# bab2min/Kiwi

Measured on AMD Instinct MI355X. Metric: sentences/sec on batched analyze(), device kernels with inputs resident in HBM (dictionary scan + lattice + Viterbi/Knlm, top-1); host-to-host rate: see e2e, higher is better.
Workload: dtype int32+f32; 1 GPU; c2-64k: 65536 synthetic sentences ({'exact_jamo': 40}), synthetic 'full' model (kiwi_amd/synth.py), Knlm, top-1; sentences_per_gpu=65536, chunks_per_gpu=65536, jamo_per_gpu=2621440, parallelism=shard1, device_bytes=9547378333, rerun_chunks=0

## Files before the change

### kiwi_amd/csrc/device_types.hpp

```cpp
#pragma once
#include <cstdint>
#include "flat_model.hpp"

namespace kamd
{
	struct DevPattern { uint32_t end, length; uint32_t tag; };
	constexpr uint32_t kSpanTag = 0x80000000u, kSpanFallback = 0x40000000u, kSpanFormMask = 0x00FFFFFFu;

	struct alignas(16) DevNode
	{
		uint32_t form;
		uint16_t startPos, endPos;
		uint16_t prev, sibling;
		uint16_t uformOff, uformLen;
		uint8_t spaceErrors;
		uint8_t nflags;
		uint16_t nPrev;
		uint32_t packOff;
		uint16_t candCnt;
		uint8_t fflags;
		uint8_t flen;
		uint16_t ownFeat;
		uint16_t pad;
	};
// ... 125 lines not shown
		const uint32_t* packBase;
		CandStatic* packs;
		const uint64_t* tokenBase;
		DevToken* tokens;
		DevChunkResult* results;
		DevPathHeader* outPaths;
		DevToken* outTokens;
		uint32_t* outCounters;
		uint32_t* wideList;
		uint8_t* expanded;
		float* unkChr;
		float* unkChrForm;
		const uint32_t* blockBits;
		uint32_t outPathCap, outTokCap;
		PosRec* posRecs; PosDesc* posDesc; uint32_t* posPrev; uint32_t* posNodeRec; uint32_t* posMask;
		uint8_t* posBig;
		uint8_t* posScratch; uint32_t* posContCounter; uint32_t posContSlots;
		uint32_t* posHandOver;
		uint8_t* bigScratch;
		uint32_t bigScratchBytes;
		uint32_t* beacon;
	};

	struct SbgDev
	{
		const uint32_t* ptrs;
		const uint32_t* keys;
		const float* comps;
		const float* discnts;
		const uint8_t* valid;
		uint32_t vocabSize; float logWindowSize;
// ... 87 lines not shown
```

### kiwi_amd/csrc/engine.hip

```cpp
#include <hip/hip_runtime.h>
#include <unistd.h>
#include <cstdio>
#include <cstring>
#include <ctime>
#include <algorithm>
#include <atomic>
#include <cstdlib>
#include <chrono>
#include <condition_variable>
#include <functional>
#include <map>
#include <mutex>
#include <numeric>
#include <stdexcept>
#include <thread>
#include "engine.hpp"
#include "pretok.hpp"
#include "hostpool.hpp"
#include "post_fast.hpp"
#include "viterbi_kernel.hpp"
#include "exact_math.hpp"
#include "cong_global.hpp"
#include "chr_freq.hpp"
#include "typo_lattice_kernel.hpp"
// ... 160 lines not shown
		uint64_t units = 0, devBytes = 0;
		std::vector<uint32_t> charOff, patOff, spOff, matchBase, nodeBase, packBase;
		std::vector<uint64_t> stateBase, tokenBase;
		PinBuf hIn; DevBuf dIn;
		DevBuf dFullMask, dZAt, dNsToPos, dPosToNs, dCflag, dMask, dMoff, dNNs, dMatchForm, dNodes, dTmpNodes, dEndPosMap, dTmpIdx, dNNodes, dWideList, dExpanded;
		struct LatClass { uint32_t i, j, need, stream; };
		std::vector<std::vector<LatClass>> latClasses; std::vector<uint32_t> latSkip; uint32_t latClassesKey = 0xFFFFFFFFu;
		DevBuf dHist;
		uint32_t slotCap = 0; uint64_t ownStates = 0;
		DevBuf dStateAt, dSlotTable; uint64_t poolStates = 0, poolUsed = 0;
		TypoOption typo;
		TypoGraphDev typoDev;
		DevBuf dTypoGraph, dTypoLast, dTypoPool, dTypoChunks, dTypoTmp, dTypoMap, dTypoNs, dTypoPs, dTypoStates, dTypoSIdx, dTypoScratch, dNodeTypo, dTypoOrder, dBlockBits, dUnkChr, dUnkChrForm;
		TypoLatView tv{};
		DevBuf dPacks, dStates, dNodeStOff, dNodeStCnt, dReach, dTokens, dResults, dOrder;
		DevBuf dPosRecs, dPosDesc, dPosPrev, dPosNodeRec, dPosMask, dPosBig;
		DevBuf dOutPaths, dOutTokens, dOutCounters; uint32_t outPathCap = 0, outTokCap = 0;
		PinBuf hOut, hOut2;
		uint64_t outBytes = 0;
		BatchView bv{}; WorkView wv{};
		const DevChunkResult* hResults = nullptr; const DevPathHeader* hPaths = nullptr; const DevToken* hTokens = nullptr; size_t hTokCount = 0;
		bool ran = false;
		hipEvent_t evDone = nullptr; bool launched = false; uint32_t launchS = 1;
		~StagedBatch()
		{
			if (evDone) (void)hipEventDestroy(evDone);
			if (prepBlocks.size() >= 64)
			{
				try { HostPool::instance().run(prepBlocks.size(), 16, hostThreads, [&](size_t i0, size_t i1, int) { for (size_t i = i0; i < i1; ++i) { PrepBlock dead = std::move(prepBlocks[i]); } }); }
				catch (...) {}
			}
// ... 427 lines not shown
		b.poolStates = tinyArenas ? 0 : slotMode ? (I.poolForced ? ownStates * I.poolFrac64 / 64 : ownStates / 4)
			: std::max<uint64_t>(ownStates * I.poolFrac64 / 64, I.poolFrac64 ? std::min<uint64_t>(ownStates, 1u << 16) : 0);
		b.ownStates = ownStates;
		const uint64_t totStates = ownStates + b.poolStates, totTokens = b.tokenBase[nC];
		b.dNsToPos.ensure(perChar * 2); b.dPosToNs.ensure(perChar * 2); b.dCflag.ensure(perChar); b.dMask.ensure(perChar * 8); b.dMoff.ensure(perChar * 4);
		b.dNNs.ensure(nC * 4 + 16); b.dMatchForm.ensure(totMatch * 4 + 16);
		b.dNodes.ensure(totNodes * sizeof(DevNode) + 16); b.dTmpNodes.ensure(totNodes * sizeof(DevNode) + 16);
		b.dEndPosMap.ensure(perChar * 4); b.dFullMask.ensure(perChar * 8); b.dZAt.ensure(perChar); b.dTmpIdx.ensure(totNodes * 4 + 16); b.dNNodes.ensure(nC * 4 + 16); b.dWideList.ensure(nC * 4 + 16); b.dExpanded.ensure(nC + 16);
		b.dPacks.ensure((size_t)b.packBase[nC] * sizeof(CandStatic) + 16);
		b.dStates.ensure(totStates * sizeof(DevState) + 16); b.dNodeStOff.ensure(totNodes * 4 + 16); b.dNodeStCnt.ensure(totNodes * 4 + 16); b.dReach.ensure(totNodes + 16);
		b.dTokens.ensure(totTokens * sizeof(DevToken) + 16); b.dResults.ensure(nC * sizeof(DevChunkResult) + 16);
		const bool posPath = I.posPath && !I.histStates();
		if (posPath)
		{
			b.dPosRecs.ensure((size_t)b.packBase[nC] * sizeof(PosRec) + 16); b.dPosDesc.ensure(totNodes * sizeof(PosDesc) + 16);
			b.dPosPrev.ensure(totNodes * 4 + 16); b.dPosNodeRec.ensure(totNodes * 4 + 16); b.dPosMask.ensure(totNodes * (b.typo.typo ? 8 : 4) + 16) ; b.dPosBig.ensure(((nC + 7) / 8 * 8) * (size_t)64 * 20 + 16);
		}
		if (I.histStates()) b.dHist.ensure(totStates * 32 + 32);
		b.outTokCap = (uint32_t)std::min<uint64_t>(totTokens, 0xFFFFFFF0ull); b.outPathCap = (uint32_t)std::min<uint64_t>((uint64_t)nC * 16 * sc, 0xFFFFFFF0ull);
		b.dOutTokens.ensure((size_t)b.outTokCap * sizeof(DevToken) + 16); b.dOutPaths.ensure((size_t)b.outPathCap * sizeof(DevPathHeader) + 16); b.dOutCounters.ensure(128);
		b.dStateAt.ensure(nC * 8 + 16); if (slotMode) b.dSlotTable.ensure((size_t)I.histSlots() * 16 + 16);
		b.devBytes = 0;
		for (const DevBuf* d : { &b.dIn, &b.dOutTokens, &b.dOutPaths, &b.dNsToPos, &b.dPosToNs, &b.dCflag, &b.dMask, &b.dMoff, &b.dMatchForm, &b.dNodes, &b.dTmpNodes, &b.dEndPosMap, &b.dTmpIdx,
			&b.dPacks, &b.dStates, &b.dHist, &b.dStateAt, &b.dSlotTable, &b.dNodeStOff, &b.dNodeStCnt, &b.dReach, &b.dTokens, &b.dResults, &b.dPosRecs, &b.dPosDesc, &b.dPosPrev, &b.dPosNodeRec, &b.dPosMask, &b.dPosBig }) b.devBytes += d->cap;

		BatchView& bv = b.bv;
		bv.nChunks = (uint32_t)nC; bv.chars = (const uint16_t*)(D + oChars); bv.cls = D + oCls; bv.script = D + oScript;
		bv.charOff = (const uint32_t*)(D + oCharOff); bv.patOff = (const uint32_t*)(D + oPatOff); bv.patterns = (const DevPattern*)(D + oPats);
		bv.spOff = (const uint32_t*)(D + oSpOff); bv.spStates = D + oSp; bv.chunkFlags = D + oFlags; bv.textOffset = (const uint32_t*)(D + oTextOff);
		bv.filtChars = chrFreq ? (const uint16_t*)(D + oFilt) : nullptr; bv.filtOff = chrFreq ? (const uint32_t*)(D + oFiltOff) : nullptr; bv.filtLen = chrFreq ? (const uint32_t*)(D + oFiltLen) : nullptr;
		WorkView& w = b.wv;
		w.nsToPos = b.dNsToPos.as<uint16_t>(); w.posToNs = b.dPosToNs.as<uint16_t>(); w.cflag = b.dCflag.as<uint8_t>();
		w.matchMask = b.dMask.as<uint64_t>(); w.matchOff = b.dMoff.as<uint32_t>(); w.nNs = b.dNNs.as<uint32_t>();
		w.matchBase = (const uint32_t*)(D + oMatchBase); w.matchForm = b.dMatchForm.as<uint32_t>();
		w.nodeBase = (const uint32_t*)(D + oNodeBase); w.nodes = b.dNodes.as<DevNode>(); w.tmpNodes = b.dTmpNodes.as<DevNode>();
		w.endPosMap = b.dEndPosMap.as<uint32_t>(); w.fullMask = b.dFullMask.as<uint64_t>(); w.zAt = b.dZAt.as<uint8_t>(); w.tmpIdx = b.dTmpIdx.as<uint16_t>(); w.nNodes = b.dNNodes.as<uint32_t>(); w.wideList = b.dWideList.as<uint32_t>(); w.expanded = b.dExpanded.as<uint8_t>();
		w.packBase = (const uint32_t*)(D + oPackBase); w.packs = b.dPacks.as<CandStatic>();
		w.stateBase = (const uint64_t*)(D + oStateBase); w.states = b.dStates.as<DevState>();
		w.stateAt = b.dStateAt.as<uint64_t>(); w.poolTop = b.poolStates ? reinterpret_cast<unsigned long long*>(b.dOutCounters.as<uint32_t>() + 16) : nullptr;
		w.poolBase = b.ownStates; w.poolCap = b.poolStates; w.slotCap = b.slotCap; w.slotTable = b.slotCap ? b.dSlotTable.as<uint64_t>() : nullptr;
		w.nodeStateOff = b.dNodeStOff.as<uint32_t>(); w.nodeStateCnt = b.dNodeStCnt.as<uint32_t>(); w.reach = b.dReach.as<uint8_t>();
		w.tokenBase = (const uint64_t*)(D + oTokenBase); w.tokens = b.dTokens.as<DevToken>(); w.results = b.dResults.as<DevChunkResult>();
		w.outTokens = b.dOutTokens.as<DevToken>(); w.outPaths = b.dOutPaths.as<DevPathHeader>(); w.outCounters = b.dOutCounters.as<uint32_t>();
		w.outTokCap = b.outTokCap; w.outPathCap = b.outPathCap;
		w.posRecs = posPath ? b.dPosRecs.as<PosRec>() : nullptr; w.posDesc = posPath ? b.dPosDesc.as<PosDesc>() : nullptr;
		w.posPrev = posPath ? b.dPosPrev.as<uint32_t>() : nullptr; w.posNodeRec = posPath ? b.dPosNodeRec.as<uint32_t>() : nullptr; w.posMask = posPath ? b.dPosMask.as<uint32_t>() : nullptr; w.posBig = posPath ? b.dPosBig.as<uint8_t>() : nullptr;
		w.posHandOver = nullptr; w.posScratch = nullptr; w.posContCounter = nullptr; w.posContSlots = 0;
		w.blockBits = nullptr;
		w.unkChr = nullptr;
		w.unkChrForm = nullptr;
		if ((b.match >> 8) & 3) { b.dUnkChr.ensure(totNodes * 4 + 16); w.unkChr = b.dUnkChr.as<float>(); }
		if (((b.match >> 8) & 3) > 1) { b.dUnkChrForm.ensure(totNodes * 4 + 16); w.unkChrForm = b.dUnkChrForm.as<float>(); }
		if (b.typo.blocked && !b.typo.blocked->empty() && b.typo.blocked->size() != (I.model.morphs.size() + 31) / 32) throw std::invalid_argument{ "kiwi_amd: blocklist bit set does not belong to this model" };
		const size_t nTempMorphs = b.pretok ? b.pretok->temps.morphs.size() : 0;
		if (!I.model.morphDialect.empty() || (nTempMorphs && b.typo.blocked && !b.typo.blocked->empty()))
		{
			std::vector<uint32_t>& bits = b.blockBitsHost;
			bits.assign((I.model.morphs.size() + 31) / 32, 0u);
			if (b.typo.blocked && !b.typo.blocked->empty()) bits = *b.typo.blocked;
			bool any = b.typo.blocked && !b.typo.blocked->empty();
			for (size_t i = 0; i < I.model.morphDialect.size(); ++i) { const uint32_t d = I.model.morphDialect[i]; if (d && !(d & b.typo.allowedDialect)) { bits[i >> 5] |= 1u << (i & 31); any = true; } }
// ... 1762 lines not shown
```

### kiwi_amd/csrc/viterbi_pos.inc

```
#if !defined(KAMD_SBG) && !defined(KAMD_CONGG)
	template<int G> struct PosCaps
	{
#ifdef KAMD_TEST_SMALL_CAPS
		static constexpr uint32_t PST_CAP = 8;
#else
		static constexpr uint32_t PST_CAP = G == 16 ? 64 : 32;
#endif
		static constexpr uint32_t PHR = G == 16 ? 32 : 16;
	};
	constexpr uint32_t PBIG_CAP = 64;
	struct PosBigItem { uint32_t keyLo, keyHi; float score, fcs; uint32_t ctx; };
	struct PosGroupCtx { uint64_t st, recs, uniq, nodeTypo; uint32_t stCap, stTop, posStart, ringTop, firstRec, retry, ofNodes, bigBase; };
	static_assert(sizeof(PosGroupCtx) == 64, "PosGroupCtx");
	template<int G> struct PosLayT
	{
		static constexpr uint32_t PST_CAP = PosCaps<G>::PST_CAP, PHR = PosCaps<G>::PHR;
		static constexpr uint32_t RBEG = 0, REND = 4 * RING, RCUM = 8 * RING;
		static constexpr uint32_t NCNT = 12 * RING;
		static constexpr uint32_t ACUR = NCNT + 4 * G, ALAST = ACUR + 32, ATMP = ALAST + 32;
		static constexpr uint32_t GCTX = ATMP + 32;
		static constexpr uint32_t RINFO = GCTX + 64;
		static constexpr uint32_t PBEST = RINFO;
		static constexpr uint32_t OVFL = RINFO + 4 * G;
		static constexpr uint32_t RECS = OVFL + 16;
		static constexpr uint32_t STSC = RECS + G * 48;
		static constexpr uint32_t STB = STSC + 4 * PST_CAP;
		static constexpr uint32_t HOTR = (STB + 2 * PST_CAP + 15) & ~15u;
// ... 2 lines not shown
		static constexpr uint32_t CTXR = TYPR + 4 * PHR, SIZE = (CTXR + 4 * PHR + 15) & ~15u;
#else
		static constexpr uint32_t CHR = TYPR + 4 * PHR, SIZE = (CHR + 8 * PHR + 15) & ~15u;
#endif
		static constexpr uint32_t ROWMAP = (64 / G) * SIZE, TOTAL = ROWMAP + 128;
	};
#if defined(KAMD_TYPO)
	constexpr uint32_t kPosLds16 = kPosKernelLdsBytes + 4 * kTypoRingExtra, kPosLds8 = kPosKernelLdsBytes8 + 8 * kTypoRingExtra;
#else
	constexpr uint32_t kPosLds16 = kPosKernelLdsBytes, kPosLds8 = kPosKernelLdsBytes8;
#endif
	static_assert(PosLayT<16>::TOTAL <= kPosLds16 && PosLayT<8>::TOTAL <= kPosLds8, "k_pos_path LDS");
	static_assert(Lay<16>::TOTAL <= kPosLds16 && Lay<16>::TOTAL <= kPosLds8, "k_pos_path LDS: the general search carrying on in the kernel");
	enum : uint32_t { PSB_PASS1 = 0x1000 };
#if defined(KAMD_POSSTATS) && defined(KAMD_HIPEMU)
	struct PosStats { std::atomic<unsigned long long> c[24]; ~PosStats() { fprintf(stderr, "[posstats] waveSteps %llu groupSteps %llu rounds %llu bigRounds %llu itemLanes %llu deadParents %llu scored %llu kept %llu multiChunkItems %llu roundsWithMulti %llu argmaxIters %llu reps %llu lmCalls %llu retries %llu rowsUsed %llu zItems %llu sockItems %llu testSteps %llu testChunks %llu\n",
		c[0].load(), c[1].load(), c[2].load(), c[3].load(), c[4].load(), c[5].load(), c[6].load(), c[7].load(), c[8].load(), c[9].load(), c[10].load(), c[11].load(), c[12].load(), c[13].load(), c[14].load(), c[15].load(), c[16].load(), c[17].load(), c[18].load()); } };
	static PosStats gPosStats;
	struct PosHist { std::atomic<unsigned long long> h[6][70]; ~PosHist() { static const char* nm[6] = { "nRec", "nodes", "newStates", "itemsPerRecord", "parentAge", "nodeDist" }; for (int a = 0; a < 6; ++a) { fprintf(stderr, "[poshist] %s:", nm[a]); for (int b = 0; b < 70; ++b) if (h[a][b].load()) fprintf(stderr, " %d:%llu", b, h[a][b].load()); fprintf(stderr, "\n"); } } };
	static PosHist gPosHist;
#define PHIST(a, v) gPosHist.h[a][(v) < 69u ? (v) : 69u]++;
#define PSTAT(k, n) gPosStats.c[k] += (n);
#else
#define PSTAT(k, n) (void)0;
#define PHIST(a, v) (void)0;
#endif

	__device__ __forceinline__ uint32_t rowOr16(uint32_t v) { v |= rowRor<8>(v); v |= rowRor<4>(v); v |= rowRor<2>(v); v |= rowRor<1>(v); return v; }
	__device__ __forceinline__ uint32_t rowMaxU16(uint32_t v)
	{
		uint32_t o;
		o = rowRor<8>(v); v = o > v ? o : v; o = rowRor<4>(v); v = o > v ? o : v; o = rowRor<2>(v); v = o > v ? o : v; o = rowRor<1>(v); v = o > v ? o : v;
// ... 70 lines not shown
		return true;
	}

	template<int G, int WPS>
	__global__ void __launch_bounds__(64, WPS) k_pos_path(ModelView M, BatchView B, WorkView W, SearchParams P, const uint32_t* chunkOrder, uint32_t nWork TYPO_ONLY(, const float* nodeTypoAll) CONG_ONLY(, CongDev CGv))
	{
		static_assert(G == 16 || G == 8, "a lane group is one DPP row or half of one");
		using PosLay = PosLayT<G>;
		constexpr uint32_t NG = 64 / G, GM = (1u << G) - 1u, PST_CAP = PosLay::PST_CAP, PHR = PosLay::PHR;
#ifdef KAMD_TYPO
		constexpr uint32_t kP = 2;
#else
		constexpr uint32_t kP = 16 / G;
#endif
		const uint32_t lane = threadIdx.x, gl = lane & (uint32_t)(G - 1), gshift = lane & (uint32_t)(64 - G), grp = lane / (uint32_t)G, lds = grp * PosLay::SIZE;
		const uint32_t il = lane & 15u, ishift = lane & 48u, irow = lane >> 4; (void)ishift;
		LDS_AS uint32_t* rBeg = ldsPtr<uint32_t>(lds + PosLay::RBEG);
		LDS_AS uint32_t* rEnd = ldsPtr<uint32_t>(lds + PosLay::REND);
		LDS_AS uint32_t* rCum = ldsPtr<uint32_t>(lds + PosLay::RCUM);
		LDS_AS uint32_t* nCnt = ldsPtr<uint32_t>(lds + PosLay::NCNT);
		LDS_AS uint32_t* aCur = ldsPtr<uint32_t>(lds + PosLay::ACUR);
		LDS_AS uint32_t* aLast = ldsPtr<uint32_t>(lds + PosLay::ALAST);
		LDS_AS uint32_t* aTmp = ldsPtr<uint32_t>(lds + PosLay::ATMP);
		LDS_AS uint32_t* gctx = ldsPtr<uint32_t>(lds + PosLay::GCTX);
		LDS_AS uint32_t* rinfo = ldsPtr<uint32_t>(lds + PosLay::RINFO);
		LDS_AS uint32_t* ovfL = ldsPtr<uint32_t>(lds + PosLay::OVFL);
		LDS_AS uint16_t* rowMap = ldsPtr<uint16_t>(PosLay::ROWMAP);
		rowMap[lane] = 0;
		auto tbit = [](LDS_AS uint32_t* a, uint32_t x) -> uint32_t { return (a[(x >> 5) & 7u] >> (x & 31u)) & 1u; };
		auto sbit = [](LDS_AS uint32_t* a, uint32_t x) { a[(x >> 5) & 7u] |= 1u << (x & 31u); };
		LDS_AS float* typR = ldsPtr<float>(lds + PosLay::TYPR);
#ifdef KAMD_CONG
		LDS_AS uint32_t* ctxR = ldsPtr<uint32_t>(lds + PosLay::CTXR);
#else
		LDS_AS uint32_t* chR = ldsPtr<uint32_t>(lds + PosLay::CHR);
#endif
		const uint32_t hotR = lds + PosLay::HOTR;
		LDS_AS float* stSc = ldsPtr<float>(lds + PosLay::STSC);
		LDS_AS uint16_t* stB = ldsPtr<uint16_t>(lds + PosLay::STB);
#define GBALLOT(p) ((uint32_t)((__ballot(p) >> gshift) & GM))
#define GSHFL(v, l) __shfl((v), (int)(l), G)
#ifdef KAMD_HIPEMU
#define WBALLOT(p) hipemu_ballot64(p)
#define WSHFL(v, l) hipemu_shfl64((v), (int)(l))
#define WREADLANE(v, l) hipemu_shfl64((v), (int)(l))
#define ISHFL16(v, l) hipemu_shfl64((v), (int)(ishift + ((uint32_t)(l) & 15u)))
#define IROR(N, v) ((uint32_t)hipemu_row_ror64((int)(v), (N)))
#define IRORF(N, v) __uint_as_float((uint32_t)hipemu_row_ror64((int)__float_as_uint(v), (N)))
#else
#define WBALLOT(p) ((unsigned long long)__ballot(p))
#define WSHFL(v, l) __shfl((v), (int)(l), 64)
#define WREADLANE(v, l) ((uint32_t)__builtin_amdgcn_readlane((int)(v), (int)(l)))
#define ISHFL16(v, l) __shfl((v), (int)(l), 16)
#define IROR(N, v) rowRor<N>(v)
#define IRORF(N, v) rowRorF<N>(v)
#endif
#define IBALLOT16(p) ((uint32_t)((WBALLOT(p) >> ishift) & 0xFFFFu))
#ifdef KAMD_POS_DEBUG
#define PBEACON(code, a, b2, c2) { if (W.beacon && mine && gl == 0) { uint32_t* bq_ = W.beacon + 64ull * chunk; __builtin_nontemporal_store((uint32_t)(code), bq_); __builtin_nontemporal_store((uint32_t)(a), bq_ + 1); __builtin_nontemporal_store((uint32_t)(b2), bq_ + 2); __builtin_nontemporal_store((uint32_t)(c2), bq_ + 3); } }
		unsigned long long tlLast = clock64(); uint32_t tlAcc[14] = { 0, 0, 0, 0, 0, 0, 0, 0, 0, 0, 0, 0, 0, 0 };
#define PTL(k) { const unsigned long long t_ = clock64(); tlAcc[k] += (uint32_t)(t_ - tlLast); tlLast = t_; }
#else
#define PBEACON(code, a, b2, c2)
#define PTL(k)
#endif
		const unsigned long long lowerMask64 = (1ull << lane) - 1ull;

		const uint32_t ci = blockIdx.x * NG + grp;
		const bool mine = ci < nWork;
		const uint32_t chunk = mine ? chunkOrder[ci] : chunkOrder[0];
		DevChunkResult* res = &W.results[chunk];
		bool active = mine && res->status == CS_OK;
		if (mine && !active && gl == 0) res->nPaths = 0;
		const bool searching = active;
		PBEACON(1, ci, 0, 0)
		const uint32_t nBase = W.nodeBase[chunk];
		const uint32_t Gn = W.nNodes[chunk];
		DevState* st = W.states + W.stateBase[chunk];
		const uint32_t stCap = (uint32_t)(W.stateBase[chunk + 1] - W.stateBase[chunk]);
		uint32_t* nodeStOff = W.nodeStateOff + nBase; uint32_t* nodeStCnt = W.nodeStateCnt + nBase; uint16_t* nodeLive = W.tmpIdx + 2ull * nBase;
		const uint8_t* uniq = B.spStates + B.spOff[chunk];
// ... 181 lines not shown
#endif
				if (active)
				{
					rinfo[gl] = pBegRp[0] | ((rqp[0] & 0xFFu) << 27);
					if (gl < nRec) { ldsStore4(lds + PosLay::RECS + 48 * gl, rec0); ldsStore4(lds + PosLay::RECS + 48 * gl + 16, rec1); ldsStore4(lds + PosLay::RECS + 48 * gl + 32, rec2); }
					if (gl == 0)
					{
						LDS_AS uint64_t* g64 = (LDS_AS uint64_t*)gctx;
						g64[0] = (uint64_t)st; g64[1] = (uint64_t)(recs + firstRec); g64[2] = (uint64_t)uniq; g64[3] = (uint64_t)nodeTypo;
						gctx[8] = stCap; gctx[9] = stTop; gctx[10] = stTop; gctx[11] = ringTop; gctx[12] = 0; gctx[13] = retry0 | (retry1 << 16);
#ifdef KAMD_CONG
						gctx[14] = ofNodes;
#else
						gctx[14] = 0;
#endif
						gctx[15] = (blockIdx.x * NG + grp) * PBIG_CAP;
						*ovfL = 0;
					}
					posStart = stTop;
				}
				PTL(1)
			}
			__syncthreads();

			for (uint32_t pass = 0; pass < kP; ++pass)
			{
			if (pass)
			{
				if (!WBALLOT(active && nRec > (uint32_t)G)) break;
				if (active)
				{
// ... 8 lines not shown
			}
			const uint32_t Qw = active ? ((kP > 1 && pass) ? Qp[kP - 1] : Qp[0]) : 0u;

			{
				uint32_t S16 = Qw;
				{ uint32_t t; t = IROR(1, S16); S16 += il >= 1 ? t : 0u; t = IROR(2, S16); S16 += il >= 2 ? t : 0u; t = IROR(4, S16); S16 += il >= 4 ? t : 0u; t = IROR(8, S16); S16 += il >= 8 ? t : 0u; }
				const uint32_t T0 = WREADLANE(S16, 15), T1 = WREADLANE(S16, 31), T2 = WREADLANE(S16, 47);
				const uint32_t Winc = S16 + (irow >= 1 ? T0 : 0u) + (irow >= 2 ? T1 : 0u) + (irow >= 3 ? T2 : 0u);
				const unsigned long long nzAll = WBALLOT(Qw != 0);
				uint32_t recDoneW = 0, baseW = 0, guardW = 0;
				while (recDoneW < 64)
				{
					const unsigned long long nz = nzAll & ~((1ull << recDoneW) - 1ull);
					if (!nz) break;
					if (++guardW > 80u) { *ovfL = 1; break; }
					const uint32_t first = (uint32_t)__ffsll((unsigned long long)nz) - 1u;
					const uint32_t Qfirst = WREADLANE(Qw, first);
					const bool bigMode = Qfirst > 16u;
					int myRow = -1; uint32_t myStart = 0, nRows = 0, myItemsRow = 0;
					if (bigMode) { recDoneW = first + 1; baseW = WREADLANE(Winc, first); }
					else
					{
						for (uint32_t b = 0; b < 4; ++b)
						{
							const bool take = lane >= recDoneW && Winc - baseW <= 16u;
							const unsigned long long tm = WBALLOT(take);
							const uint32_t n = (uint32_t)__popcll(tm);
							if (!n) break;
							if (take) { myRow = (int)b; myStart = Winc - Qw - baseW; }
							const uint32_t it = WREADLANE(Winc, recDoneW + n - 1) - baseW;
							if (irow == b) myItemsRow = it;
							baseW += it; recDoneW += n; nRows = b + 1;
							if (recDoneW >= 64) break;
						}
					}
					PTL(2)
					if (lane == 0) { PSTAT(2, 1) PSTAT(3, bigMode ? 1 : 0) PSTAT(14, bigMode ? 4 : nRows) }
					const uint32_t q = bigMode ? lane : il;
					bool valid; uint32_t recLane, local, lastK = 0;
					if (!bigMode)
					{
						if (myRow >= 0 && Qw) rowMap[16 * (uint32_t)myRow + myStart] = (uint16_t)((lane | (myStart << 8) | ((Qw - 1u) << 12)) + 1u);
						__syncthreads();
						valid = irow < nRows && il < myItemsRow;
						uint32_t e = rowMap[lane];
						rowMap[lane] = 0;
						{ uint32_t o;
						  o = IROR(1, e); e = (e == 0 && il >= 1) ? o : e;
						  o = IROR(2, e); e = (e == 0 && il >= 2) ? o : e;
						  o = IROR(4, e); e = (e == 0 && il >= 4) ? o : e;
						  o = IROR(8, e); e = (e == 0 && il >= 8) ? o : e; }
						e = e ? e - 1u : 0u;
						recLane = valid ? (e & 0xFFu) : lane;
						local = valid ? il - ((e >> 8) & 15u) : 0u;
						lastK = valid ? ((e >> 8) & 15u) + (e >> 12) : il;
					}
					else { valid = lane < Qfirst; recLane = valid ? first : lane; local = lane; }
					const uint32_t startK = q - local;
					const uint32_t owner = recLane / (uint32_t)G, k = recLane & (uint32_t)(G - 1), ldsO = owner * PosLay::SIZE;
					const uint4 g0 = ldsLoad4(ldsO + PosLay::GCTX), g1 = ldsLoad4(ldsO + PosLay::GCTX + 16), g2 = ldsLoad4(ldsO + PosLay::GCTX + 32), g3 = ldsLoad4(ldsO + PosLay::GCTX + 48);
					DevState* stO = reinterpret_cast<DevState*>((uint64_t)g0.x | ((uint64_t)g0.y << 32));
					const uint8_t* uniqO = reinterpret_cast<const uint8_t*>((uint64_t)g1.x | ((uint64_t)g1.y << 32));
					const float* nodeTypoO = reinterpret_cast<const float*>((uint64_t)g1.z | ((uint64_t)g1.w << 32)); (void)nodeTypoO;
					const uint32_t stCapO = g2.x, stTopO = g2.y, posStartO = g2.z, ringTopO = g2.w;
					const uint32_t retry0O = g3.y & 0xFFFFu, retry1O = g3.y >> 16, bigBaseO = g3.w;
					CONG_ONLY(const uint32_t ofNodesO = g3.z;)
					const uint32_t ri = ldsPtr<uint32_t>(ldsO + PosLay::RINFO)[k];
					const uint32_t pBegK = ri & 0x7FFFFFFu, R = ri >> 27;
					const uint32_t hotRO = ldsO + PosLay::HOTR;
					LDS_AS float* typRO = ldsPtr<float>(ldsO + PosLay::TYPR);
#ifdef KAMD_CONG
					LDS_AS uint32_t* ctxRO = ldsPtr<uint32_t>(ldsO + PosLay::CTXR);
#else
					LDS_AS uint32_t* chRO = ldsPtr<uint32_t>(ldsO + PosLay::CHR);
#endif
					LDS_AS float* stScO = ldsPtr<float>(ldsO + PosLay::STSC);
					LDS_AS uint16_t* stBO = ldsPtr<uint16_t>(ldsO + PosLay::STB);
					uint4 ra = make_uint4(0, 0, 0, 0), rb = ra, rc = ra;
					if (valid) { ra = ldsLoad4(ldsO + PosLay::RECS + 48 * k); rb = ldsLoad4(ldsO + PosLay::RECS + 48 * k + 16); rc = ldsLoad4(ldsO + PosLay::RECS + 48 * k + 32); }
					Cand c;
// ... 5 lines not shown
					const uint8_t ownKind = (uint8_t)(rc.z >> 16), nflags = (uint8_t)(rc.z >> 24);
					const uint32_t nl = (rc.w >> 8) & 0xFFu;
					const bool spaceBefore = nflags & NF_SPACE_BEFORE;
					const bool isZ = (rc.w & PR_Z) != 0;
					uint32_t p = local, r = 0;
					if (R > 1) { p = local / R; r = local % R; }

					PTL(3)
					float cand = 0, firstChunk = 0, rTypo = 0; int32_t lmNode = 0; uint8_t rootKey = 0, sp = 0;
					CONG_ONLY(uint32_t ctx = 0;)
					CONG_ONLY(uint32_t pctx = 0;)
#ifndef KAMD_CONG
					uint32_t pch1 = 0, pch2 = 0, nch1 = 0, nch2 = 0;
#endif
					if (valid) PSTAT(4, 1)
					if (valid)
					{
						const uint32_t pidx = pBegK + p, slot = pidx & (PHR - 1);
						PHIST(4, ringTopO - pidx)
						Hot ps;
						if (ringTopO - pidx <= PHR)
						{
							const uint4 a = ldsLoad4(hotRO + 16 * slot);
							ps.lmNode = (int32_t)a.x; ps.accScore = __uint_as_float(a.y); ps.w2 = a.z; ps.w3 = a.w;
							rTypo = typRO[slot];
#ifdef KAMD_CONG
							pctx = ctxRO[slot];
#else
							pch1 = chRO[2 * slot]; pch2 = chRO[2 * slot + 1];
#endif
						}
						else
						{
							ps = loadHot(stO, pidx);
							rTypo = stO[pidx].accTypoCost;
#ifdef KAMD_CONG
							pctx = stO[pidx].pad0;
#else
							const uint2 pc = *reinterpret_cast<const uint2*>(&stO[pidx].pad0); pch1 = pc.x; pch2 = pc.y;
#endif
						}
						const bool single = c.single();
						const uint8_t ctag = c.tag(), csock = c.socket();
						uint32_t firstWid = c.firstWid; bool widReplaced = false;
#ifdef KAMD_POS_DEBUG
						if (ps.accScore == 12345.678f && c.additional == 9876.5f) tlAcc[0] += 1;
						PTL(12)
#endif
// ... 97 lines not shown
#endif
							sp = ps.spState();
							rootKey = ps.rootId();
							if (c.quoteOrBullet())
							{
								if (rootKey == COMMON_ROOT) sp = uniqO[r];
								else if (r != 0) { valid = false; break; }
							}
							const float rs = ruleScore(c, ps.prevFlags(), sp);
							cand = cand + rs; firstChunk = firstChunk + rs;
							if (c.ruleBits & RB_DIALECT) { cand = cand - P.dialectCost; firstChunk = firstChunk - P.dialectCost; }
							sp = nextSpState(c, sp);
						} while (0);
					}
					PTL(4)
					if (valid) PSTAT(7, 1)
					const uint64_t rKey = valid ? ((uint64_t)(uint32_t)lmNode | ((uint64_t)sp << 32) | ((uint64_t)rootKey << 40) | ((uint64_t)recLane << 48)) : KINVALID;
					const float rScore = cand, rFcs = firstChunk;

					auto emitState = [&](uint32_t pos, bool ring, int32_t wNode, uint8_t wSp, uint8_t wRoot, float wscore, float wfcs, float wtyp, uint32_t wx1, uint32_t wx2, uint32_t wl)
					{
						const uint32_t rslot = pos & (PHR - 1);
						uint32_t parent = pBegK + wl, wr = 0;
						if (R != 1) { parent = pBegK + wl / R; wr = wl % R; }
						const uint32_t rel = pos - posStartO;
						if (isZ)
						{
							const uint4* ps4 = reinterpret_cast<const uint4*>(stO + parent);
							const uint4 a = ps4[0], b2 = ps4[1], c2 = ps4[2];
							const uint16_t lfMorph = (uint16_t)c.chunkOff; const uint8_t nmPrevFlags = (uint8_t)(c.chunkOff >> 16); const bool newMorphSocket = (c.chunkOff >> 24) & 1u;
// ... 44 lines not shown
							ctxRO[rslot] = wx1;
#else
							chRO[2 * rslot] = wx1; chRO[2 * rslot + 1] = wx2;
#endif
						}
#ifdef KAMD_CONG
						(void)wx2;
#else
						*reinterpret_cast<uint2*>(&stO[pos].pad0) = make_uint2(wx1, wx2);
#endif
						stScO[rel] = wscore;
						stBO[rel] = (uint16_t)((newRoot == COMMON_ROOT ? 0u : newRoot + 1u) | (c.socket() ? (uint32_t)SB_MORPH_SOCKET : 0u) | (stSocket ? (uint32_t)SB_STATE_SOCKET : 0u)
							| (nl << 8) | ((rc.w & PR_PASS1) ? (uint32_t)PSB_PASS1 : 0u));
					};
					const uint32_t keyLo = (uint32_t)rKey, keyHi = (uint32_t)(rKey >> 32);
					bool rep; float best, wfcs, wtyp; uint32_t wl, wx1, wx2, wNodeU, wHi;
					if (!bigMode)
					{
						rep = false; best = rScore; uint32_t qw = q;
						const uint32_t recMask = ((2u << (lastK - startK)) - 1u) << startK;
						bool un = valid;
						while (WBALLOT(un))
						{
							if (lane == 0) PSTAT(10, 1)
							const uint32_t mine = IBALLOT16(un) & recMask;
							const uint32_t f = mine ? (uint32_t)__ffs((int)mine) - 1u : q;
							const uint32_t kLo = ISHFL16(keyLo, f), kHi = ISHFL16(keyHi, f);
							const bool match = un & (keyLo == kLo) & (keyHi == kHi);
							float bs = match ? rScore : -3.0e38f; uint32_t bi = q;
#define KAMD_POS_SEG(N) { const float os = IRORF(N, bs); const uint32_t oi = IROR(N, bi); const bool take = (q >= startK + N) & (os >= bs); bs = take ? os : bs; bi = take ? oi : bi; }
							KAMD_POS_SEG(1) KAMD_POS_SEG(2) KAMD_POS_SEG(4) KAMD_POS_SEG(8)
#undef KAMD_POS_SEG
							const float rb = ISHFL16(bs, lastK); const uint32_t rq = ISHFL16(bi, lastK);
							if (match && q == f) { rep = true; best = rb; qw = rq; }
							un = un && !match;
						}
						PTL(5)
						wfcs = ISHFL16(rFcs, qw);
						wtyp = ISHFL16(rTypo, qw);
#ifdef KAMD_CONG
						wx1 = ISHFL16(ctx, qw); wx2 = 0;
#else
						wx1 = nch1; wx2 = nch2;
#endif
						wl = qw - startK; wNodeU = (uint32_t)lmNode; wHi = keyHi;
					}
					else
					{
						PosBigItem* big = reinterpret_cast<PosBigItem*>(W.posBig) + bigBaseO;
						if (lane < Qfirst)
						{
							PosBigItem it; it.keyLo = keyLo; it.keyHi = keyHi; it.score = rScore; it.fcs = rFcs;
#ifdef KAMD_CONG
							it.ctx = ctx;
#else
							it.ctx = 0;
#endif
							big[lane] = it;
						}
						__syncthreads();
						rep = false; best = 0; uint32_t qw = lane;
						if (lane < Qfirst && (keyLo & keyHi) != 0xFFFFFFFFu)
						{
							rep = true; bool have = false;
							for (uint32_t j = 0; j < Qfirst; ++j)
							{
								if (big[j].keyLo != keyLo || big[j].keyHi != keyHi) continue;
								if (j < lane) { rep = false; break; }
								const float sj = big[j].score;
								if (!have || sj > best) { best = sj; qw = j; have = true; }
							}
						}
						wfcs = 0; wtyp = 0; wx1 = 0; wx2 = 0;
						if (rep)
						{
							wfcs = big[qw].fcs;
							wtyp = stO[pBegK + (R > 1 ? qw / R : qw)].accTypoCost;
#ifdef KAMD_CONG
							wx1 = big[qw].ctx;
#else
							if (!isZ) { const uint2 nc = *reinterpret_cast<const uint2*>(M.lmChain + 2 * (size_t)keyLo); wx1 = nc.x; wx2 = nc.y; }
#endif
						}
						wl = qw; wNodeU = keyLo; wHi = keyHi;
						__syncthreads();
					}
					uint32_t myRank = 0, myAdd = 0, ownerAdd = 0;
					for (uint32_t g2i = 0; g2i < NG; ++g2i)
					{
						const unsigned long long bg = WBALLOT(rep && owner == g2i);
						if (owner == g2i) { myRank = (uint32_t)__popcll(bg & lowerMask64); ownerAdd = (uint32_t)__popcll(bg); }
						if (grp == g2i) myAdd = (uint32_t)__popcll(bg);
					}
					if (rep) PSTAT(11, 1)
					if (rep)
					{
						const uint32_t pos = stTopO + myRank;
						if (pos < stCapO && pos - posStartO < PST_CAP) emitState(pos, pos + PHR >= stTopO + ownerAdd, (int32_t)wNodeU, (uint8_t)wHi, (uint8_t)(wHi >> 8), best, wfcs, wtyp, wx1, wx2, wl);
						else ldsPtr<uint32_t>(ldsO + PosLay::OVFL)[0] = 1;
					}
					stTop += myAdd;
					ringTop = stTop > ringTop ? stTop : ringTop;
					if (gl == 0 && myAdd) { gctx[9] = stTop; gctx[11] = ringTop; }
					PTL(6)
					__syncthreads();
				}
// ... 216 lines not shown
		bool cont = false;
		uint32_t slot = 0xFFFFFFFFu;
		if (W.posScratch)
		{
			if (handOver) { if (gl == 0) slot = atomicAdd(W.posContCounter, 1u); slot = GSHFL(slot, 0); }
			cont = handOver && slot < W.posContSlots;
		}
		if constexpr (G == 8)
		{
			const unsigned long long cm = WBALLOT(cont && gl == 0);
			if (cm)
			{
				__syncthreads();
				LDS_AS uint32_t* lst = ldsPtr<uint32_t>(PosLay::ROWMAP);
				static_assert(Lay<16>::TOTAL <= PosLayT<8>::ROWMAP && 3 * 4 * (64 / 8) <= 128, "list of the chunks carried on");
				if (cont && gl == 0) { const uint32_t at = (uint32_t)__popcll(cm & lowerMask64); lst[3 * at] = chunk; lst[3 * at + 1] = stopAt; lst[3 * at + 2] = slot; }
				const uint32_t nH = (uint32_t)__popcll(cm);
				LDS_AS float* lb = ldsPtr<float>(Lay<16>::LB);
				for (uint32_t t = lane; t < 2 * T_MAX + 1; t += 64)
				{
					float v = 0;
					if (t == 2 * T_MAX) v = 5.f;
					else if (t < T_MAX) { if (t == T_NNP || t == T_NP || t == T_IC) v = -1; else if (t == T_SB) v = -3; }
					else { const uint8_t r = (uint8_t)(t - T_MAX); v = (isEClass(r) || isJClass(r) || isSuffixTag(r) || r == T_VCP) ? -1.f : 0.f; }
					lb[t] = v;
				}
				__syncthreads();
#ifdef KAMD_HIPEMU
				hipemu_set_width(16);
#endif
				for (uint32_t base = 0; base < nH; base += 4)
// ... 42 lines not shown
				const PosKernArgs A{ M, B, W, P, chunkOrder, nWork TYPO_ONLY(, nodeTypoAll) CONG_ONLY(, CGv) };
				cont = continueChunk(&A, chunk, gl, grp, slot, stopAt & 0xFFFFFFu, W.posScratch, chunkOrder, nWork);
#else
				cont = continueChunk(chunk, gl, grp, slot, stopAt & 0xFFFFFFu, W.posScratch, chunkOrder, nWork);
#endif
				if (cont && gl == 0) res->pad = kPosChunkDone | (stopAt & 0xFF000000u);
			}
		}
		if (handOver && !cont && gl == 0) { res->pad = stopAt; *W.posHandOver = 1; }
		}
#undef GBALLOT
#undef GSHFL
#undef WBALLOT
#undef WSHFL
#undef WREADLANE
#undef ISHFL16
#undef IROR
#undef IRORF
#undef IBALLOT16
#undef PBEACON
#undef PTL
#undef PSTAT
#undef PHIST
	}
#endif
```

Measured before the change: 13.20 million sentences/s.

## Pack records wave-wide and drop global big-record scratch path in POS search

Replaces the per-16-lane row packing with a single 64-lane packing of records per round. Candidate dedup now runs as a wave-wide segmented max, using row rotates plus cross-row readlane carries. This removes the separate bigMode path that staged items in global scratch and scanned them with an O(Q^2) loop, along with its buffer allocation. Lane-rank computation switches to mbcnt. In exchange, every dedup iteration pays extra readlanes and 64-wide shuffles, and records longer than 64 items now trip the overflow path instead of being handled.

```diff
diff --git a/kiwi_amd/csrc/device_types.hpp b/kiwi_amd/csrc/device_types.hpp
--- a/kiwi_amd/csrc/device_types.hpp
+++ b/kiwi_amd/csrc/device_types.hpp
@@ -163,7 +163,6 @@
 		const uint32_t* blockBits;
 		uint32_t outPathCap, outTokCap;
 		PosRec* posRecs; PosDesc* posDesc; uint32_t* posPrev; uint32_t* posNodeRec; uint32_t* posMask;
-		uint8_t* posBig;
 		uint8_t* posScratch; uint32_t* posContCounter; uint32_t posContSlots;
 		uint32_t* posHandOver;
 		uint8_t* bigScratch;
diff --git a/kiwi_amd/csrc/engine.hip b/kiwi_amd/csrc/engine.hip
--- a/kiwi_amd/csrc/engine.hip
+++ b/kiwi_amd/csrc/engine.hip
@@ -198,7 +198,7 @@
 		DevBuf dTypoGraph, dTypoLast, dTypoPool, dTypoChunks, dTypoTmp, dTypoMap, dTypoNs, dTypoPs, dTypoStates, dTypoSIdx, dTypoScratch, dNodeTypo, dTypoOrder, dBlockBits, dUnkChr, dUnkChrForm;
 		TypoLatView tv{};
 		DevBuf dPacks, dStates, dNodeStOff, dNodeStCnt, dReach, dTokens, dResults, dOrder;
-		DevBuf dPosRecs, dPosDesc, dPosPrev, dPosNodeRec, dPosMask, dPosBig;
+		DevBuf dPosRecs, dPosDesc, dPosPrev, dPosNodeRec, dPosMask;
 		DevBuf dOutPaths, dOutTokens, dOutCounters; uint32_t outPathCap = 0, outTokCap = 0;
 		PinBuf hOut, hOut2;
 		uint64_t outBytes = 0;
@@ -656,7 +656,7 @@
 		if (posPath)
 		{
 			b.dPosRecs.ensure((size_t)b.packBase[nC] * sizeof(PosRec) + 16); b.dPosDesc.ensure(totNodes * sizeof(PosDesc) + 16);
-			b.dPosPrev.ensure(totNodes * 4 + 16); b.dPosNodeRec.ensure(totNodes * 4 + 16); b.dPosMask.ensure(totNodes * (b.typo.typo ? 8 : 4) + 16) ; b.dPosBig.ensure(((nC + 7) / 8 * 8) * (size_t)64 * 20 + 16);
+			b.dPosPrev.ensure(totNodes * 4 + 16); b.dPosNodeRec.ensure(totNodes * 4 + 16); b.dPosMask.ensure(totNodes * (b.typo.typo ? 8 : 4) + 16) ;
 		}
 		if (I.histStates()) b.dHist.ensure(totStates * 32 + 32);
 		b.outTokCap = (uint32_t)std::min<uint64_t>(totTokens, 0xFFFFFFF0ull); b.outPathCap = (uint32_t)std::min<uint64_t>((uint64_t)nC * 16 * sc, 0xFFFFFFF0ull);
@@ -664,7 +664,7 @@
 		b.dStateAt.ensure(nC * 8 + 16); if (slotMode) b.dSlotTable.ensure((size_t)I.histSlots() * 16 + 16);
 		b.devBytes = 0;
 		for (const DevBuf* d : { &b.dIn, &b.dOutTokens, &b.dOutPaths, &b.dNsToPos, &b.dPosToNs, &b.dCflag, &b.dMask, &b.dMoff, &b.dMatchForm, &b.dNodes, &b.dTmpNodes, &b.dEndPosMap, &b.dTmpIdx,
-			&b.dPacks, &b.dStates, &b.dHist, &b.dStateAt, &b.dSlotTable, &b.dNodeStOff, &b.dNodeStCnt, &b.dReach, &b.dTokens, &b.dResults, &b.dPosRecs, &b.dPosDesc, &b.dPosPrev, &b.dPosNodeRec, &b.dPosMask, &b.dPosBig }) b.devBytes += d->cap;
+			&b.dPacks, &b.dStates, &b.dHist, &b.dStateAt, &b.dSlotTable, &b.dNodeStOff, &b.dNodeStCnt, &b.dReach, &b.dTokens, &b.dResults, &b.dPosRecs, &b.dPosDesc, &b.dPosPrev, &b.dPosNodeRec, &b.dPosMask }) b.devBytes += d->cap;
 
 		BatchView& bv = b.bv;
 		bv.nChunks = (uint32_t)nC; bv.chars = (const uint16_t*)(D + oChars); bv.cls = D + oCls; bv.script = D + oScript;
@@ -686,7 +686,7 @@
 		w.outTokens = b.dOutTokens.as<DevToken>(); w.outPaths = b.dOutPaths.as<DevPathHeader>(); w.outCounters = b.dOutCounters.as<uint32_t>();
 		w.outTokCap = b.outTokCap; w.outPathCap = b.outPathCap;
 		w.posRecs = posPath ? b.dPosRecs.as<PosRec>() : nullptr; w.posDesc = posPath ? b.dPosDesc.as<PosDesc>() : nullptr;
-		w.posPrev = posPath ? b.dPosPrev.as<uint32_t>() : nullptr; w.posNodeRec = posPath ? b.dPosNodeRec.as<uint32_t>() : nullptr; w.posMask = posPath ? b.dPosMask.as<uint32_t>() : nullptr; w.posBig = posPath ? b.dPosBig.as<uint8_t>() : nullptr;
+		w.posPrev = posPath ? b.dPosPrev.as<uint32_t>() : nullptr; w.posNodeRec = posPath ? b.dPosNodeRec.as<uint32_t>() : nullptr; w.posMask = posPath ? b.dPosMask.as<uint32_t>() : nullptr;
 		w.posHandOver = nullptr; w.posScratch = nullptr; w.posContCounter = nullptr; w.posContSlots = 0;
 		w.blockBits = nullptr;
 		w.unkChr = nullptr;
diff --git a/kiwi_amd/csrc/viterbi_pos.inc b/kiwi_amd/csrc/viterbi_pos.inc
--- a/kiwi_amd/csrc/viterbi_pos.inc
+++ b/kiwi_amd/csrc/viterbi_pos.inc
@@ -9,8 +9,7 @@
 		static constexpr uint32_t PHR = G == 16 ? 32 : 16;
 	};
 	constexpr uint32_t PBIG_CAP = 64;
-	struct PosBigItem { uint32_t keyLo, keyHi; float score, fcs; uint32_t ctx; };
-	struct PosGroupCtx { uint64_t st, recs, uniq, nodeTypo; uint32_t stCap, stTop, posStart, ringTop, firstRec, retry, ofNodes, bigBase; };
+	struct PosGroupCtx { uint64_t st, recs, uniq, nodeTypo; uint32_t stCap, stTop, posStart, ringTop, firstRec, retry, ofNodes, pad; };
 	static_assert(sizeof(PosGroupCtx) == 64, "PosGroupCtx");
 	template<int G> struct PosLayT
 	{
@@ -43,8 +42,8 @@
 	static_assert(Lay<16>::TOTAL <= kPosLds16 && Lay<16>::TOTAL <= kPosLds8, "k_pos_path LDS: the general search carrying on in the kernel");
 	enum : uint32_t { PSB_PASS1 = 0x1000 };
 #if defined(KAMD_POSSTATS) && defined(KAMD_HIPEMU)
-	struct PosStats { std::atomic<unsigned long long> c[24]; ~PosStats() { fprintf(stderr, "[posstats] waveSteps %llu groupSteps %llu rounds %llu bigRounds %llu itemLanes %llu deadParents %llu scored %llu kept %llu multiChunkItems %llu roundsWithMulti %llu argmaxIters %llu reps %llu lmCalls %llu retries %llu rowsUsed %llu zItems %llu sockItems %llu testSteps %llu testChunks %llu\n",
-		c[0].load(), c[1].load(), c[2].load(), c[3].load(), c[4].load(), c[5].load(), c[6].load(), c[7].load(), c[8].load(), c[9].load(), c[10].load(), c[11].load(), c[12].load(), c[13].load(), c[14].load(), c[15].load(), c[16].load(), c[17].load(), c[18].load()); } };
+	struct PosStats { std::atomic<unsigned long long> c[24]; ~PosStats() { fprintf(stderr, "[posstats] waveSteps %llu groupSteps %llu rounds %llu bigRounds %llu itemLanes %llu deadParents %llu scored %llu kept %llu multiChunkItems %llu roundsWithMulti %llu argmaxIters %llu reps %llu lmCalls %llu retries %llu rowsUsed %llu zItems %llu sockItems %llu testSteps %llu testChunks %llu straddlingRecords %llu arenaParentRounds %llu\n",
+		c[0].load(), c[1].load(), c[2].load(), c[3].load(), c[4].load(), c[5].load(), c[6].load(), c[7].load(), c[8].load(), c[9].load(), c[10].load(), c[11].load(), c[12].load(), c[13].load(), c[14].load(), c[15].load(), c[16].load(), c[17].load(), c[18].load(), c[19].load(), c[20].load()); } };
 	static PosStats gPosStats;
 	struct PosHist { std::atomic<unsigned long long> h[6][70]; ~PosHist() { static const char* nm[6] = { "nRec", "nodes", "newStates", "itemsPerRecord", "parentAge", "nodeDist" }; for (int a = 0; a < 6; ++a) { fprintf(stderr, "[poshist] %s:", nm[a]); for (int b = 0; b < 70; ++b) if (h[a][b].load()) fprintf(stderr, " %d:%llu", b, h[a][b].load()); fprintf(stderr, "\n"); } } };
 	static PosHist gPosHist;
@@ -145,7 +144,7 @@
 		constexpr uint32_t kP = 16 / G;
 #endif
 		const uint32_t lane = threadIdx.x, gl = lane & (uint32_t)(G - 1), gshift = lane & (uint32_t)(64 - G), grp = lane / (uint32_t)G, lds = grp * PosLay::SIZE;
-		const uint32_t il = lane & 15u, ishift = lane & 48u, irow = lane >> 4; (void)ishift;
+		const uint32_t il = lane & 15u, irow = lane >> 4;
 		LDS_AS uint32_t* rBeg = ldsPtr<uint32_t>(lds + PosLay::RBEG);
 		LDS_AS uint32_t* rEnd = ldsPtr<uint32_t>(lds + PosLay::REND);
 		LDS_AS uint32_t* rCum = ldsPtr<uint32_t>(lds + PosLay::RCUM);
@@ -175,18 +174,17 @@
 #define WBALLOT(p) hipemu_ballot64(p)
 #define WSHFL(v, l) hipemu_shfl64((v), (int)(l))
 #define WREADLANE(v, l) hipemu_shfl64((v), (int)(l))
-#define ISHFL16(v, l) hipemu_shfl64((v), (int)(ishift + ((uint32_t)(l) & 15u)))
+#define WBELOW(m) ((uint32_t)__popcll((unsigned long long)(m) & ((1ull << lane) - 1ull)))
 #define IROR(N, v) ((uint32_t)hipemu_row_ror64((int)(v), (N)))
 #define IRORF(N, v) __uint_as_float((uint32_t)hipemu_row_ror64((int)__float_as_uint(v), (N)))
 #else
 #define WBALLOT(p) ((unsigned long long)__ballot(p))
 #define WSHFL(v, l) __shfl((v), (int)(l), 64)
 #define WREADLANE(v, l) ((uint32_t)__builtin_amdgcn_readlane((int)(v), (int)(l)))
-#define ISHFL16(v, l) __shfl((v), (int)(l), 16)
+#define WBELOW(m) __builtin_amdgcn_mbcnt_hi((uint32_t)((unsigned long long)(m) >> 32), __builtin_amdgcn_mbcnt_lo((uint32_t)(m), 0u))
 #define IROR(N, v) rowRor<N>(v)
 #define IRORF(N, v) rowRorF<N>(v)
 #endif
-#define IBALLOT16(p) ((uint32_t)((WBALLOT(p) >> ishift) & 0xFFFFu))
 #ifdef KAMD_POS_DEBUG
 #define PBEACON(code, a, b2, c2) { if (W.beacon && mine && gl == 0) { uint32_t* bq_ = W.beacon + 64ull * chunk; __builtin_nontemporal_store((uint32_t)(code), bq_); __builtin_nontemporal_store((uint32_t)(a), bq_ + 1); __builtin_nontemporal_store((uint32_t)(b2), bq_ + 2); __builtin_nontemporal_store((uint32_t)(c2), bq_ + 3); } }
 		unsigned long long tlLast = clock64(); uint32_t tlAcc[14] = { 0, 0, 0, 0, 0, 0, 0, 0, 0, 0, 0, 0, 0, 0 };
@@ -195,7 +193,6 @@
 #define PBEACON(code, a, b2, c2)
 #define PTL(k)
 #endif
-		const unsigned long long lowerMask64 = (1ull << lane) - 1ull;
 
 		const uint32_t ci = blockIdx.x * NG + grp;
 		const bool mine = ci < nWork;
@@ -407,7 +404,6 @@
 #else
 						gctx[14] = 0;
 #endif
-						gctx[15] = (blockIdx.x * NG + grp) * PBIG_CAP;
 						*ovfL = 0;
 					}
 					posStart = stTop;
@@ -446,56 +442,42 @@
 					const unsigned long long nz = nzAll & ~((1ull << recDoneW) - 1ull);
 					if (!nz) break;
 					if (++guardW > 80u) { *ovfL = 1; break; }
-					const uint32_t first = (uint32_t)__ffsll((unsigned long long)nz) - 1u;
-					const uint32_t Qfirst = WREADLANE(Qw, first);
-					const bool bigMode = Qfirst > 16u;
-					int myRow = -1; uint32_t myStart = 0, nRows = 0, myItemsRow = 0;
-					if (bigMode) { recDoneW = first + 1; baseW = WREADLANE(Winc, first); }
-					else
-					{
-						for (uint32_t b = 0; b < 4; ++b)
-						{
-							const bool take = lane >= recDoneW && Winc - baseW <= 16u;
-							const unsigned long long tm = WBALLOT(take);
-							const uint32_t n = (uint32_t)__popcll(tm);
-							if (!n) break;
-							if (take) { myRow = (int)b; myStart = Winc - Qw - baseW; }
-							const uint32_t it = WREADLANE(Winc, recDoneW + n - 1) - baseW;
-							if (irow == b) myItemsRow = it;
-							baseW += it; recDoneW += n; nRows = b + 1;
-							if (recDoneW >= 64) break;
-						}
-					}
+					const bool take = lane >= recDoneW && Winc - baseW <= 64u;
+					const uint32_t nTake = (uint32_t)__popcll(WBALLOT(take));
+					if (!nTake) { *ovfL = 1; break; }
+					const uint32_t nItems = WREADLANE(Winc, recDoneW + nTake - 1) - baseW;
+					const uint32_t myStart = Winc - Qw - baseW;
+					if (take && Qw) rowMap[myStart] = (uint16_t)((lane | ((Qw - 1u) << 6)) + 1u);
+					if (lane == 0) { PSTAT(2, 1) PSTAT(14, (nItems + 15u) >> 4) }
+					if (take && Qw) { if (Qw > 16u) PSTAT(3, 1) else if ((myStart >> 4) != ((myStart + Qw - 1u) >> 4)) PSTAT(19, 1) }
+					baseW += nItems; recDoneW += nTake;
 					PTL(2)
-					if (lane == 0) { PSTAT(2, 1) PSTAT(3, bigMode ? 1 : 0) PSTAT(14, bigMode ? 4 : nRows) }
-					const uint32_t q = bigMode ? lane : il;
-					bool valid; uint32_t recLane, local, lastK = 0;
-					if (!bigMode)
-					{
-						if (myRow >= 0 && Qw) rowMap[16 * (uint32_t)myRow + myStart] = (uint16_t)((lane | (myStart << 8) | ((Qw - 1u) << 12)) + 1u);
-						__syncthreads();
-						valid = irow < nRows && il < myItemsRow;
-						uint32_t e = rowMap[lane];
-						rowMap[lane] = 0;
-						{ uint32_t o;
-						  o = IROR(1, e); e = (e == 0 && il >= 1) ? o : e;
-						  o = IROR(2, e); e = (e == 0 && il >= 2) ? o : e;
-						  o = IROR(4, e); e = (e == 0 && il >= 4) ? o : e;
-						  o = IROR(8, e); e = (e == 0 && il >= 8) ? o : e; }
-						e = e ? e - 1u : 0u;
-						recLane = valid ? (e & 0xFFu) : lane;
-						local = valid ? il - ((e >> 8) & 15u) : 0u;
-						lastK = valid ? ((e >> 8) & 15u) + (e >> 12) : il;
-					}
-					else { valid = lane < Qfirst; recLane = valid ? first : lane; local = lane; }
-					const uint32_t startK = q - local;
+					__syncthreads();
+					const uint32_t q = lane;
+					bool valid = lane < nItems;
+					uint32_t e = rowMap[lane];
+					rowMap[lane] = 0;
+					e = e ? ((e - 1u) | (lane << 12) | 0x80000000u) : 0u;
+					{ uint32_t o;
+					  o = IROR(1, e); e = (e == 0 && il >= 1) ? o : e;
+					  o = IROR(2, e); e = (e == 0 && il >= 2) ? o : e;
+					  o = IROR(4, e); e = (e == 0 && il >= 4) ? o : e;
+					  o = IROR(8, e); e = (e == 0 && il >= 8) ? o : e;
+					  const uint32_t t0 = WREADLANE(e, 15), t1 = WREADLANE(e, 31), t2 = WREADLANE(e, 47);
+					  const uint32_t c2 = t1 ? t1 : t0, c3 = t2 ? t2 : c2;
+					  o = irow == 1 ? t0 : irow == 2 ? c2 : irow == 3 ? c3 : 0u;
+					  e = e == 0 ? o : e; }
+					const uint32_t recLane = valid ? (e & 63u) : lane;
+					const uint32_t startK = valid ? ((e >> 12) & 63u) : lane;
+					const uint32_t lastK = valid ? startK + ((e >> 6) & 63u) : lane;
+					const uint32_t local = q - startK;
 					const uint32_t owner = recLane / (uint32_t)G, k = recLane & (uint32_t)(G - 1), ldsO = owner * PosLay::SIZE;
 					const uint4 g0 = ldsLoad4(ldsO + PosLay::GCTX), g1 = ldsLoad4(ldsO + PosLay::GCTX + 16), g2 = ldsLoad4(ldsO + PosLay::GCTX + 32), g3 = ldsLoad4(ldsO + PosLay::GCTX + 48);
 					DevState* stO = reinterpret_cast<DevState*>((uint64_t)g0.x | ((uint64_t)g0.y << 32));
 					const uint8_t* uniqO = reinterpret_cast<const uint8_t*>((uint64_t)g1.x | ((uint64_t)g1.y << 32));
 					const float* nodeTypoO = reinterpret_cast<const float*>((uint64_t)g1.z | ((uint64_t)g1.w << 32)); (void)nodeTypoO;
 					const uint32_t stCapO = g2.x, stTopO = g2.y, posStartO = g2.z, ringTopO = g2.w;
-					const uint32_t retry0O = g3.y & 0xFFFFu, retry1O = g3.y >> 16, bigBaseO = g3.w;
+					const uint32_t retry0O = g3.y & 0xFFFFu, retry1O = g3.y >> 16;
 					CONG_ONLY(const uint32_t ofNodesO = g3.z;)
 					const uint32_t ri = ldsPtr<uint32_t>(ldsO + PosLay::RINFO)[k];
 					const uint32_t pBegK = ri & 0x7FFFFFFu, R = ri >> 27;
@@ -531,6 +513,9 @@
 					uint32_t pch1 = 0, pch2 = 0, nch1 = 0, nch2 = 0;
 #endif
 					if (valid) PSTAT(4, 1)
+#if defined(KAMD_POSSTATS) && defined(KAMD_HIPEMU)
+					bool arenaParent = false;
+#endif
 					if (valid)
 					{
 						const uint32_t pidx = pBegK + p, slot = pidx & (PHR - 1);
@@ -549,6 +534,9 @@
 						}
 						else
 						{
+#if defined(KAMD_POSSTATS) && defined(KAMD_HIPEMU)
+							arenaParent = true;
+#endif
 							ps = loadHot(stO, pidx);
 							rTypo = stO[pidx].accTypoCost;
 #ifdef KAMD_CONG
@@ -676,6 +664,9 @@
 						} while (0);
 					}
 					PTL(4)
+#if defined(KAMD_POSSTATS) && defined(KAMD_HIPEMU)
+					{ const unsigned long long am = WBALLOT(arenaParent); if (lane == 0 && am) PSTAT(20, 1) }
+#endif
 					if (valid) PSTAT(7, 1)
 					const uint64_t rKey = valid ? ((uint64_t)(uint32_t)lmNode | ((uint64_t)sp << 32) | ((uint64_t)rootKey << 40) | ((uint64_t)recLane << 48)) : KINVALID;
 					const float rScore = cand, rFcs = firstChunk;
@@ -750,82 +741,44 @@
 							| (nl << 8) | ((rc.w & PR_PASS1) ? (uint32_t)PSB_PASS1 : 0u));
 					};
 					const uint32_t keyLo = (uint32_t)rKey, keyHi = (uint32_t)(rKey >> 32);
-					bool rep; float best, wfcs, wtyp; uint32_t wl, wx1, wx2, wNodeU, wHi;
-					if (!bigMode)
-					{
-						rep = false; best = rScore; uint32_t qw = q;
-						const uint32_t recMask = ((2u << (lastK - startK)) - 1u) << startK;
-						bool un = valid;
-						while (WBALLOT(un))
-						{
-							if (lane == 0) PSTAT(10, 1)
-							const uint32_t mine = IBALLOT16(un) & recMask;
-							const uint32_t f = mine ? (uint32_t)__ffs((int)mine) - 1u : q;
-							const uint32_t kLo = ISHFL16(keyLo, f), kHi = ISHFL16(keyHi, f);
-							const bool match = un & (keyLo == kLo) & (keyHi == kHi);
-							float bs = match ? rScore : -3.0e38f; uint32_t bi = q;
-#define KAMD_POS_SEG(N) { const float os = IRORF(N, bs); const uint32_t oi = IROR(N, bi); const bool take = (q >= startK + N) & (os >= bs); bs = take ? os : bs; bi = take ? oi : bi; }
-							KAMD_POS_SEG(1) KAMD_POS_SEG(2) KAMD_POS_SEG(4) KAMD_POS_SEG(8)
+					bool rep = false; float best = rScore; uint32_t qw = q;
+					const uint32_t recLen1 = lastK - startK;
+					bool un = valid;
+					unsigned long long um = WBALLOT(un);
+					for (uint32_t guardK = 0; um && guardK < 64u; ++guardK)
+					{
+						if (lane == 0) PSTAT(10, 1)
+						const unsigned long long mine = (um >> startK) & ((2ull << recLen1) - 1ull);
+						const uint32_t f = mine ? startK + (uint32_t)__ffsll(mine) - 1u : q;
+						const uint32_t kLo = WSHFL(keyLo, f), kHi = WSHFL(keyHi, f);
+						const bool match = un & (keyLo == kLo) & (keyHi == kHi);
+						float bs = match ? rScore : -3.0e38f; uint32_t bi = q;
+#define KAMD_POS_SEG(N) { const float os = IRORF(N, bs); const uint32_t oi = IROR(N, bi); const bool tk = (il >= N) & (q >= startK + N) & (os >= bs); bs = tk ? os : bs; bi = tk ? oi : bi; }
+						KAMD_POS_SEG(1) KAMD_POS_SEG(2) KAMD_POS_SEG(4) KAMD_POS_SEG(8)
 #undef KAMD_POS_SEG
-							const float rb = ISHFL16(bs, lastK); const uint32_t rq = ISHFL16(bi, lastK);
-							if (match && q == f) { rep = true; best = rb; qw = rq; }
-							un = un && !match;
-						}
-						PTL(5)
-						wfcs = ISHFL16(rFcs, qw);
-						wtyp = ISHFL16(rTypo, qw);
-#ifdef KAMD_CONG
-						wx1 = ISHFL16(ctx, qw); wx2 = 0;
-#else
-						wx1 = nch1; wx2 = nch2;
-#endif
-						wl = qw - startK; wNodeU = (uint32_t)lmNode; wHi = keyHi;
-					}
-					else
-					{
-						PosBigItem* big = reinterpret_cast<PosBigItem*>(W.posBig) + bigBaseO;
-						if (lane < Qfirst)
-						{
-							PosBigItem it; it.keyLo = keyLo; it.keyHi = keyHi; it.score = rScore; it.fcs = rFcs;
-#ifdef KAMD_CONG
-							it.ctx = ctx;
-#else
-							it.ctx = 0;
-#endif
-							big[lane] = it;
-						}
-						__syncthreads();
-						rep = false; best = 0; uint32_t qw = lane;
-						if (lane < Qfirst && (keyLo & keyHi) != 0xFFFFFFFFu)
-						{
-							rep = true; bool have = false;
-							for (uint32_t j = 0; j < Qfirst; ++j)
-							{
-								if (big[j].keyLo != keyLo || big[j].keyHi != keyHi) continue;
-								if (j < lane) { rep = false; break; }
-								const float sj = big[j].score;
-								if (!have || sj > best) { best = sj; qw = j; have = true; }
-							}
-						}
-						wfcs = 0; wtyp = 0; wx1 = 0; wx2 = 0;
-						if (rep)
-						{
-							wfcs = big[qw].fcs;
-							wtyp = stO[pBegK + (R > 1 ? qw / R : qw)].accTypoCost;
-#ifdef KAMD_CONG
-							wx1 = big[qw].ctx;
-#else
-							if (!isZ) { const uint2 nc = *reinterpret_cast<const uint2*>(M.lmChain + 2 * (size_t)keyLo); wx1 = nc.x; wx2 = nc.y; }
-#endif
-						}
-						wl = qw; wNodeU = keyLo; wHi = keyHi;
-						__syncthreads();
-					}
+#define KAMD_POS_SEGX(B) { const float os = __uint_as_float(WREADLANE(__float_as_uint(bs), B)); const uint32_t oi = WREADLANE(bi, B); const bool tk = (irow == (B + 1u) / 16u) & (startK <= B) & (os >= bs); bs = tk ? os : bs; bi = tk ? oi : bi; }
+						KAMD_POS_SEGX(15u) KAMD_POS_SEGX(31u) KAMD_POS_SEGX(47u)
+#undef KAMD_POS_SEGX
+						const float rb = WSHFL(bs, lastK); const uint32_t rq = WSHFL(bi, lastK);
+						if (match && q == f) { rep = true; best = rb; qw = rq; }
+						un = un && !match;
+						um = WBALLOT(un);
+					}
+					if (um) ldsPtr<uint32_t>(ldsO + PosLay::OVFL)[0] = 1;
+					PTL(5)
+					const float wfcs = WSHFL(rFcs, qw);
+					const float wtyp = WSHFL(rTypo, qw);
+#ifdef KAMD_CONG
+					const uint32_t wx1 = WSHFL(ctx, qw), wx2 = 0;
+#else
+					const uint32_t wx1 = nch1, wx2 = nch2;
+#endif
+					const uint32_t wl = qw - startK, wNodeU = (uint32_t)lmNode, wHi = keyHi;
 					uint32_t myRank = 0, myAdd = 0, ownerAdd = 0;
 					for (uint32_t g2i = 0; g2i < NG; ++g2i)
 					{
 						const unsigned long long bg = WBALLOT(rep && owner == g2i);
-						if (owner == g2i) { myRank = (uint32_t)__popcll(bg & lowerMask64); ownerAdd = (uint32_t)__popcll(bg); }
+						if (owner == g2i) { myRank = WBELOW(bg); ownerAdd = (uint32_t)__popcll(bg); }
 						if (grp == g2i) myAdd = (uint32_t)__popcll(bg);
 					}
 					if (rep) PSTAT(11, 1)
@@ -1072,7 +1025,7 @@
 				__syncthreads();
 				LDS_AS uint32_t* lst = ldsPtr<uint32_t>(PosLay::ROWMAP);
 				static_assert(Lay<16>::TOTAL <= PosLayT<8>::ROWMAP && 3 * 4 * (64 / 8) <= 128, "list of the chunks carried on");
-				if (cont && gl == 0) { const uint32_t at = (uint32_t)__popcll(cm & lowerMask64); lst[3 * at] = chunk; lst[3 * at + 1] = stopAt; lst[3 * at + 2] = slot; }
+				if (cont && gl == 0) { const uint32_t at = WBELOW(cm); lst[3 * at] = chunk; lst[3 * at + 1] = stopAt; lst[3 * at + 2] = slot; }
 				const uint32_t nH = (uint32_t)__popcll(cm);
 				LDS_AS float* lb = ldsPtr<float>(Lay<16>::LB);
 				for (uint32_t t = lane; t < 2 * T_MAX + 1; t += 64)
@@ -1145,10 +1098,9 @@
 #undef WBALLOT
 #undef WSHFL
 #undef WREADLANE
-#undef ISHFL16
+#undef WBELOW
 #undef IROR
 #undef IRORF
-#undef IBALLOT16
 #undef PBEACON
 #undef PTL
 #undef PSTAT
```

Result: faster. 14.06 million sentences/s, median of 6 (+6.5%).
